# benanil/CLRayTracer

Hardware: AMD Instinct MI355X
Metric: Mrays/s (primary + traced secondary rays), ms/frame at 1920x1080 (higher is better)
Workload: dtype f32

## Files before the change

clraytracer_amd/_lib.py:

```python
import ctypes as C
import os

import numpy as np

os.environ.setdefault("GPU_MAX_HW_QUEUES", "8")

_HERE = os.path.dirname(os.path.abspath(__file__))
ROOT = os.path.dirname(_HERE)
HIP_SO = os.path.join(_HERE, "csrc", "libcrt_hip.so")
HOST_SO = os.path.join(_HERE, "host", "libcrt_host.so")


class CrtTraceArgs(C.Structure):
    _fields_ = [("cameraPos", C.c_float * 3), ("time", C.c_float), ("numMeshes", C.c_uint32), ("sunAngle", C.c_float)]


class CrtFrameStats(C.Structure):
    _fields_ = [("frames", C.c_uint64), ("sumMs", C.c_double * 4), ("extentMs", C.c_double), ("firstFrameMs", C.c_double)]


class CrtCounters(C.Structure):
    _fields_ = [(n, C.c_uint64) for n in ("rays", "primary", "secondary", "hits", "misses", "traversals", "pops",
                                          "innerVisits", "triTests", "capHits", "stackOverflows", "maxStack",
                                          "shadowRays", "shadowHits")]
# ... 22 lines not shown

HIP_API = {
    "crt_init": (C.c_int, [C.c_int, C.c_int, C.c_int]),
    "crt_init_devices": (C.c_int, [C.POINTER(C.c_int), C.c_int, C.c_int, C.c_int]),
    "crt_init_gpus": (C.c_int, [C.c_int, C.c_int, C.c_int]),
    "crt_num_devices": (C.c_int, []),
    "crt_peer_access": (C.c_int, [C.c_int]),
    "crt_gather_path": (C.c_char_p, []),
    "crt_get_cull_range": (C.c_int, [_fp, C.c_int, _fp, _fp, C.POINTER(C.c_uint64)]),
    "crt_debug_staggered_frames": (C.c_int, [C.POINTER(C.c_uint64)]),
    "crt_debug_inject_failure": (C.c_int, [C.c_int]),
    "crt_debug_last_kernel": (C.c_int, [C.c_char_p, C.c_size_t]),
    "crt_debug_last_gather": (C.c_int, [C.POINTER(C.c_uint64), C.POINTER(C.c_int)]),
    "crt_debug_build_stats": (C.c_int, [C.POINTER(C.c_uint32), C.POINTER(C.c_uint32)]),
    "crt_debug_tlas_stats": (C.c_int, [C.POINTER(C.c_uint64), C.POINTER(C.c_uint32), C.POINTER(C.c_uint32)]),
    "crt_debug_measure_clock": (C.c_int, [C.c_int, C.POINTER(C.c_double)]),
    "crt_shutdown": (C.c_int, []),
    "crt_resize": (C.c_int, [C.c_int, C.c_int]),
    "crt_set_row_bands": (C.c_int, [C.c_int, C.c_int, C.c_int]),
    "crt_row_owner": (C.c_int, [C.c_int, C.c_int, C.c_int]),
    "crt_band_plan": (C.c_int, [C.c_int, C.c_int, C.c_int, C.c_int, C.POINTER(C.c_int)]),
    "crt_upload_triangles": (C.c_int, [_vp, _sz, _sz]),
    "crt_upload_bvh_nodes": (C.c_int, [_vp, _sz, _sz]),
    "crt_upload_bvh_roots": (C.c_int, [_vp, _sz, _sz]),
    "crt_upload_materials": (C.c_int, [_vp, _sz, _sz]),
    "crt_upload_texture_table": (C.c_int, [_vp, _sz]),
    "crt_upload_texels": (C.c_int, [_vp, _sz, _sz]),
    "crt_upload_instances": (C.c_int, [_vp, _sz, _sz]),
    "crt_build_bvh": (C.c_int, [_sz, _vp, C.c_int, _sz, _sz, C.POINTER(C.c_uint32)]),
    "crt_download_triangles": (C.c_int, [_vp, _sz, _sz]),
# ... 148 lines not shown
```

clraytracer_amd/csrc/crt_device.h:

```cpp
#pragma once
#include <hip/hip_runtime.h>
#include <hip/hip_fp16.h>
#include <stdint.h>
#include "../../include/crt_types.h"

#define CRT_LEAF_BIT 0x80000000u
#define CRT_TOP_BIT 0x40000000u
#define CRT_BLOCK 64
#ifndef CRT_WAVES_PER_SIMD
#define CRT_WAVES_PER_SIMD 8
#endif
#define CRT_WAVES_PER_SIMD_COUNT 6
typedef uint32_t __attribute__((address_space(3))) * crt_lds_u32_ptr;
typedef float crt_f32x4 __attribute__((ext_vector_type(4)));
typedef const crt_f32x4 __attribute__((address_space(4)))* crt_const_f32x4_ptr;
typedef const crt_f32x4 __attribute__((address_space(3)))* crt_lds_f32x4_ptr;
#ifndef CRT_LDS_SLOTS
#define CRT_LDS_SLOTS 20
#endif
#define CRT_MAX_PARK 5
#define CRT_OVF_SLOTS_MAX (CRT_STACK_DEPTH - (CRT_LDS_SLOTS - CRT_MAX_PARK))
#define CRT_OVF_WORDS_PER_BLOCK ((size_t)CRT_OVF_SLOTS_MAX * CRT_BLOCK)
template <int PARK, int SLOTS = CRT_LDS_SLOTS, bool TOP = false>
struct CrtStackT {
    static constexpr bool kTop = TOP;
    static constexpr int kLds = SLOTS - PARK;
    static_assert(PARK >= 0 && PARK <= CRT_MAX_PARK && kLds >= 1 && kLds <= CRT_STACK_DEPTH && CRT_STACK_DEPTH - kLds <= CRT_OVF_SLOTS_MAX, "LDS slots");
    crt_lds_u32_ptr lds;
    uint32_t* ovf;
    crt_lds_f32x4_ptr top;
    uint32_t vblock;
    __device__ __forceinline__ uint32_t* overflow_slot(int k) const
    {
        uint32_t lane = threadIdx.x & 63;
        asm volatile("" : "+v"(lane));
        return ovf + ((size_t)(TOP ? vblock : blockIdx.x) * CRT_OVF_SLOTS_MAX + (size_t)k) * CRT_BLOCK + lane;
    }
    __device__ __forceinline__ void write(int slot, uint32_t v) const
    {
        const int s = slot & (CRT_STACK_DEPTH - 1);
        if (kLds >= CRT_STACK_DEPTH || __ballot(s >= kLds) == 0) { lds[s * 64] = v; return; }
        if (kLds >= CRT_STACK_DEPTH || s < kLds) lds[s * 64] = v;
        else *overflow_slot(s - kLds) = v;
    }
    __device__ __forceinline__ uint32_t read(int slot) const
    {
        const int s = slot & (CRT_STACK_DEPTH - 1);
        if (kLds >= CRT_STACK_DEPTH || __ballot(s >= kLds) == 0) return lds[s * 64];
        if (kLds >= CRT_STACK_DEPTH || s < kLds) return lds[s * 64];
        return *overflow_slot(s - kLds);
    }
    __device__ __forceinline__ crt_lds_f32x4_ptr top_record(uint32_t k) const { return top + k * 4; }
    __device__ __forceinline__ void park(int k, uint32_t v) const { lds[(kLds + k) * 64] = v; }
    __device__ __forceinline__ uint32_t parked(int k) const { return lds[(kLds + k) * 64]; }
};
typedef CrtStackT<0> CrtStack;
#ifndef CRT_SPLIT_BETA
#define CRT_SPLIT_BETA 1.2f
#endif
#ifndef CRT_SPLIT_BETA_ASYNC
#define CRT_SPLIT_BETA_ASYNC 2.0f
#endif
#define CRT_MAX_SPLIT 96
#ifndef CRT_MAX_SPLIT_PIPELINED
#define CRT_MAX_SPLIT_PIPELINED 8
#endif
#define CRT_TILE 8

struct CrtTlasNode { float4 sphere; uint32_t left, right, pad0, pad1; };
// ... 9 lines not shown
    const uint32_t* __restrict__ rootRefs;
    uint32_t* stackOverflow;
    const CrtMeshInstance* __restrict__ instances;
    const struct CrtDevInstance* __restrict__ devInstances;
    const float4* __restrict__ instBounds;
    const CrtMaterial* __restrict__ materials;
    const CrtTexture* __restrict__ textures;
    const uint32_t* __restrict__ texels;
    int numTexels;
    uint32_t numInstances;
    const CrtTlasNode* __restrict__ tlas;
    uint32_t tlasNodes;
    const uint32_t* __restrict__ alwaysList;
    uint32_t numAlways;
    const float4* __restrict__ topPairs;
};

struct CrtFrame {
    float invView[16];
    float invProj[16];
    float camPos[3];
    float lightY, lightZ;
    int width, height;
    int tilesX;
    int ownedTileRows;
    int gridBlocks;
    int tileRowsPerBand;
    int rank, nRanks;
    int slotsPerXcd;
    const uint32_t* order;
// ... 132 lines not shown
{
    CrtDevInstance I;
    const uint32_t inst0 = (uint32_t)__builtin_amdgcn_readfirstlane((int)inst);
    if (__ballot(inst != inst0) == 0) {
        const crt_const_f32x4_ptr p = (crt_const_f32x4_ptr)(table + inst0);
        const crt_f32x4 a = p[0], b = p[1], c = p[2], e = p[3];
        I.r0 = make_float4(a.x, a.y, a.z, a.w); I.r1 = make_float4(b.x, b.y, b.z, b.w);
        I.r2 = make_float4(c.x, c.y, c.z, c.w); I.r3 = make_float4(e.x, e.y, e.z, e.w);
    } else {
        const CrtDevInstance* ip = table + inst;
        I.r0 = ip->r0; I.r1 = ip->r1; I.r2 = ip->r2; I.r3 = ip->r3;
    }
    return I;
}

template <bool COUNT>
struct Traversal {
    v3 mo, md, inv;
    Triout tr;
    int sp, prot, inters;
    uint32_t ref, curInst;
    bool active;

    __device__ __forceinline__ void reset()
    {
        mo = mk3(0.f, 0.f, 0.f); md = mo; inv = mo;
        tr.t = 0.f; tr.u = 0.f; tr.v = 0.f; tr.tri = 0;
        sp = 0; prot = 0; inters = 0; ref = 0; curInst = 0; active = false;
    }
    __device__ __forceinline__ bool at_inner() const { return active && !(ref & CRT_LEAF_BIT); }
    __device__ __forceinline__ bool at_leaf() const { return active && (ref & CRT_LEAF_BIT); }

    __device__ __forceinline__ void finish(Closest& c)
    {
        if (inters) { c.hitInstance = (int)curInst; c.hit = tr; c.distance = tr.t; c.anyHit = 1; }
        active = false;
    }
    template <class STK>
    __device__ __forceinline__ void pop_next(const STK& stack, Closest& c, LaneCounters& lc)
    {
        const bool nonEmpty = sp > 0, canPop = nonEmpty && prot < CRT_MAX_POPS;
        prot += nonEmpty ? 1 : 0;
        if (COUNT) { if (nonEmpty && !canPop) lc.capHits++; if (canPop) lc.pops++; }
        if (canPop) { --sp; ref = stack.read(sp); }
        else {
            const bool keep = inters != 0;
            c.hitInstance = keep ? (int)curInst : c.hitInstance; c.distance = keep ? tr.t : c.distance; c.anyHit = keep ? 1 : c.anyHit;
            c.hit.t = keep ? tr.t : c.hit.t; c.hit.u = keep ? tr.u : c.hit.u; c.hit.v = keep ? tr.v : c.hit.v; c.hit.tri = keep ? tr.tri : c.hit.tri;
            active = false;
        }
    }
    template <bool TOP = false>
    __device__ __forceinline__ void enter(const CrtDevScene& S, uint32_t inst, v3 o, v3 d, float bestSoFar, LaneCounters& lc)
    {
        curInst = inst;
        const CrtDevInstance I = load_instance(S.devInstances, inst);
        mo = xform_xyz(I, o.x, o.y, o.z, 1.0f);
        md = xform_xyz(I, d.x, d.y, d.z, 0.0f);
        inv = mk3(1.0f / md.x, 1.0f / md.y, 1.0f / md.z);
        tr.t = bestSoFar; tr.tri = 0; tr.u = 0.0f; tr.v = 0.0f;
        ref = __float_as_uint(TOP ? I.r2.w : I.r0.w);
        sp = 0; prot = 1; inters = 0; active = true;
        if (COUNT) { lc.traversals++; lc.pops++; }
    }
    template <class STK>
    __device__ __forceinline__ void inner(const CrtDevScene& S, const STK& stack, Closest& c, LaneCounters& lc)
    {
        float dist1, dist2;
        uint32_t nearRef, farRef;
        const uint32_t ref0 = (uint32_t)__builtin_amdgcn_readfirstlane((int)ref);
        if (__ballot(ref != ref0) == 0) {
            const crt_const_f32x4_ptr q = (STK::kTop && (ref0 & CRT_TOP_BIT)) ? (crt_const_f32x4_ptr)(S.topPairs + (size_t)(ref0 & 0xFFFFu) * 4)
                                                                             : (crt_const_f32x4_ptr)(S.pairs + (size_t)ref0 * 4);
            const crt_f32x4 a = q[0], b = q[1], c4 = q[2], e = q[3];
            dist1 = intersect_aabb(mo, inv, make_float4(a.x, a.y, a.z, a.w), make_float4(b.x, b.y, b.z, b.w), tr.t);
            dist2 = intersect_aabb(mo, inv, make_float4(c4.x, c4.y, c4.z, c4.w), make_float4(e.x, e.y, e.z, e.w), tr.t);
            nearRef = __float_as_uint(a.w); farRef = __float_as_uint(c4.w);
#ifndef CRT_TOP_NO_LDS_PATH
#define CRT_TOP_NO_LDS_PATH 0
#endif
// ... 6 lines not shown
        } else {
            const float4* p = (STK::kTop && (ref & CRT_TOP_BIT)) ? S.topPairs + (size_t)(ref & 0xFFFFu) * 4 : S.pairs + (size_t)ref * 4;
            const float4 lmin = p[0], lmax = p[1], rmin = p[2], rmax = p[3];
            dist1 = intersect_aabb(mo, inv, lmin, lmax, tr.t);
            dist2 = intersect_aabb(mo, inv, rmin, rmax, tr.t);
            nearRef = __float_as_uint(lmin.w); farRef = __float_as_uint(rmin.w);
        }
        if (COUNT) lc.innerVisits++;
        {
            const bool sw = dist1 > dist2;
            const float d1 = sw ? dist2 : dist1, d2 = sw ? dist1 : dist2;
            const uint32_t r1 = sw ? farRef : nearRef, r2 = sw ? nearRef : farRef;
            dist1 = d1; dist2 = d2; nearRef = r1; farRef = r2;
        }
        if (dist2 != 1e30f) {
            if (COUNT) { if (sp >= CRT_STACK_DEPTH) lc.stackOverflows++; }
            stack.write(sp, farRef);
            sp++;
            if (COUNT) { if ((uint32_t)sp > lc.maxStack) lc.maxStack = (uint32_t)sp; }
        }
        if (dist1 == 1e30f) pop_next(stack, c, lc);
        else ref = nearRef;
    }
    template <bool ANYHIT, class STK>
    __device__ __forceinline__ void leaf(const CrtDevScene& S, const STK& stack, Closest& c, LaneCounters& lc)
    {
        const uint32_t first = ref & 0x00FFFFFFu;
        uint32_t n = (ref >> 24) & 0x7Fu;
        if (n == 0) n = S.bigLeaf[first];
        for (uint32_t i = first, end = first + n; i < end; ++i) {
            if (COUNT) lc.triTests++;
            const float* __restrict__ hot = S.triHot + (size_t)i * 9;
            inters |= intersect_triangle(mo, md, mk3(hot[0], hot[1], hot[2]), mk3(hot[3], hot[4], hot[5]), mk3(hot[6], hot[7], hot[8]), tr, i);
            if (ANYHIT) { if (inters) break; }
        }
        if (ANYHIT && inters) finish(c);
        else pop_next(stack, c, lc);
    }
};

__device__ __forceinline__ bool sphere_culls(const float4 bs, v3 o, v3 d, float dd)
{
    const v3 oc = mk3(bs.x - o.x, bs.y - o.y, bs.z - o.z);
    const float oc2 = dot3(oc, oc), b = dot3(oc, d);
    const float r2 = bs.w * bs.w * 1.0201f + 4e-6f * oc2;
    return (bs.w >= 0.0f) & ((oc2 * dd - b * b > r2 * dd) | ((b < 0.0f) & (oc2 > r2)));
}

template <bool COUNT, bool DEFER_COUNT = false>
__device__ __forceinline__ unsigned long long candidate_mask(const CrtDevScene& S, v3 o, v3 d, uint32_t base, uint32_t cnt, LaneCounters& lc)
{
    const float dd = dot3(d, d);
// ... 48 lines not shown
    uint32_t node = 0; int sp = 0;
    for (;;) {
        const CrtTlasNode nd = S.tlas[node];
        bool descend = false;
        if (!sphere_culls(nd.sphere, o, d, dd)) {
            if (nd.left & CRT_TLAS_LEAF) {
                const uint32_t i = nd.left & 0xFFFFu;
                if (i < S.numInstances) ok = candidate_list_add(stack, n, i) && ok;
            } else { stack.write(sp, nd.right); sp++; node = nd.left; descend = true; }
        }
        if (!descend) { if (sp == 0) break; --sp; node = stack.read(sp); }
    }
    return ok;
}

template <bool COUNT, bool ITERS, bool ANYHIT, class STK>
__device__ __forceinline__ void trip_steps(const CrtDevScene& S, const STK& stack, Traversal<COUNT>& T, Closest& c, LaneCounters& lc, bool done)
{
    if (!done && T.at_inner()) {
        if (ITERS) { lc.rays++; if (first_active_lane()) lc.innerVisits++; }
        T.inner(S, stack, c, lc);
    }
    if (!done && T.at_leaf()) {
        if (ITERS) {
            if (first_active_lane()) lc.triTests++;
            uint32_t n = (T.ref >> 24) & 0x7Fu; if (n == 0) n = S.bigLeaf[T.ref & 0x00FFFFFFu];
            for (int off = 32; off > 0; off >>= 1) { const uint32_t o2 = (uint32_t)__shfl_xor((int)n, off, 64); n = o2 > n ? o2 : n; }
            if (first_active_lane()) lc.misses += n;
        }
        T.template leaf<ANYHIT>(S, stack, c, lc);
    }
    if (!done && T.at_inner()) {
        if (ITERS) { if (first_active_lane()) lc.hits++; }
        T.inner(S, stack, c, lc);
    }
}

template <bool COUNT, bool ITERS = false, bool ANYHIT = false, bool TLAS = false, class STK = CrtStack>
__device__ __forceinline__ Closest closest_hit(const CrtDevScene& S, v3 o, v3 d, const STK& stack, LaneCounters& lc)
{
    Closest c = no_hit();
    Traversal<COUNT> T; T.reset();

    if constexpr (TLAS) {
        static_assert(!TLAS || STK::kLds <= CRT_LDS_SLOTS - CRT_TLAS_PARK, "the candidate list needs CRT_TLAS_PARK parked slots");
        uint32_t listed = 0;
        const bool fits = tlas_candidates(S, o, d, stack, listed);
        if (__ballot(!fits) == 0) {
            int prev = -1;
            if (COUNT && !ANYHIT) { const uint32_t culled = S.numInstances - listed; lc.traversals += culled; lc.pops += culled; lc.innerVisits += culled; lc.culled += culled; }
            bool done = false;
            for (;;) {
                const bool wEnter = !done && !T.active;
                const bool wInner = !done && T.at_inner();
                const bool wLeaf = !done && T.at_leaf();
                if (__ballot(wEnter || wInner || wLeaf) == 0) break;
                if (wEnter) {
                    const uint32_t k = (ANYHIT && c.anyHit) ? 0xFFFFu : candidate_list_next(stack, prev);
                    if (k == 0xFFFFu) {
                        done = true;
                        if (COUNT && ANYHIT && !c.anyHit) { const uint32_t n = S.numInstances - (uint32_t)(prev + 1); lc.traversals += n; lc.pops += n; lc.innerVisits += n; lc.culled += n; }
                    } else {
                        if (COUNT && ANYHIT) { const uint32_t n = k - (uint32_t)(prev + 1); lc.traversals += n; lc.pops += n; lc.innerVisits += n; lc.culled += n; }
                        prev = (int)k;
                        T.template enter<STK::kTop>(S, k, o, d, c.distance, lc);
                    }
                }
                trip_steps<COUNT, false, ANYHIT>(S, stack, T, c, lc, done);
            }
            return c;
        }
    }

    for (uint32_t base = 0; base < S.numInstances; base += 64) {
        const uint32_t cnt = (S.numInstances - base) < 64u ? (S.numInstances - base) : 64u;
        unsigned long long cand = candidate_mask<COUNT, ANYHIT>(S, o, d, base, cnt, lc);
        unsigned long long culledLeft = (COUNT && ANYHIT) ? (~cand & (cnt == 64u ? ~0ull : ((1ull << cnt) - 1ull))) : 0ull;
        bool done = ANYHIT && c.anyHit;
        for (;;) {
            const bool wEnter = !done && !T.active;
            const bool wInner = !done && T.at_inner();
            const bool wLeaf = !done && T.at_leaf();
            if (__ballot(wEnter || wInner || wLeaf) == 0) break;
// ... 3 lines not shown
                else if (cand == 0) {
                    done = true;
                    if (COUNT && ANYHIT) { const uint32_t n = (uint32_t)__popcll(culledLeft); lc.traversals += n; lc.pops += n; lc.innerVisits += n; lc.culled += n; culledLeft = 0; }
                } else {
                    if (ITERS) { if (first_active_lane()) lc.traversals++; }
                    const uint32_t k = (uint32_t)__ffsll((long long)cand) - 1u;
                    cand &= cand - 1;
                    if (COUNT && ANYHIT) {
                        const unsigned long long below = culledLeft & ((1ull << k) - 1ull);
                        const uint32_t n = (uint32_t)__popcll(below);
                        lc.traversals += n; lc.pops += n; lc.innerVisits += n; lc.culled += n; culledLeft &= ~below;
                    }
                    T.template enter<STK::kTop>(S, base + k, o, d, c.distance, lc);
                }
            }
            trip_steps<COUNT, ITERS, ANYHIT>(S, stack, T, c, lc, done);
        }
    }
    return c;
}

__device__ __forceinline__ int clamp_texel(int idx, int n) { return idx < 0 ? 0 : (idx >= n ? n - 1 : idx); }

__device__ __noinline__ int sample_skybox(v3 d, int texW, int texH)
{
    const double PI = 3.14159265358979323846;
    float at = (float)(atan2((double)d.x, (double)(-d.z)) / PI);
    float ac = (float)(acos((double)d.y) / PI);
    int theta = f2i((at * 0.5f) * (float)texW);
    int phi = f2i(ac * (float)texH);
    return (int)((uint32_t)phi * (uint32_t)texW + (uint32_t)(theta + 2));
// ... 128 lines not shown
```

clraytracer_amd/csrc/crt_instances.h:

```cpp
#pragma once
namespace {

int cache_root_nodes();
void rebuild_instance_master(uint32_t dirtyFirst = 0, uint32_t dirtyCount = CRT_MAX_INSTANCES, bool everything = true);

int rebuild_bvh_layout()
{
    HIPCHK(hipMemsetAsync(g.err, 0, sizeof(int), g.stream));
    if (g.nodeCount) {
        crt_relayout_nodes<<<(g.nodeCount + 255) / 256, 256, 0, g.stream>>>(g.rawNodes, g.nodeCount, (uint32_t)g.triCap, g.pairs, g.bigLeaf, g.err);
        HIPCHK(hipGetLastError());
    }
    crt_make_root_refs<<<(CRT_MAX_MESHES + 255) / 256, 256, 0, g.stream>>>(g.rawNodes, g.nodeCount, (uint32_t)g.triCap, g.roots, g.numRoots, g.rootRefs, g.bigLeaf, g.err);
    HIPCHK(hipGetLastError());
    {
        const uint32_t perMesh = g.numRoots ? (uint32_t)CRT_TOP_PAIRS / g.numRoots : 0u;
        crt_build_top_kernel<<<1, CRT_MAX_MESHES, 0, g.stream>>>(g.pairs, g.rootRefs, g.numRoots, perMesh, g.topPairs, g.topRootRefs);
        HIPCHK(hipGetLastError());
    }
    int err = 0;
    HIPCHK(hipMemcpyAsync(&err, g.err, sizeof(int), hipMemcpyDeviceToHost, g.stream));
    HIPCHK(hipStreamSynchronize(g.stream));
    g.sceneValid = (err == 0);
    if (err) return CRT_E_BAD_ARGUMENT;
    RCCHK(cache_root_nodes());
    rebuild_instance_master();
    return CRT_OK;
}

bool invert4(const double m[16], double out[16])
{
    double a[4][8];
    for (int r = 0; r < 4; ++r) for (int c = 0; c < 4; ++c) { a[r][c] = m[r * 4 + c]; a[r][4 + c] = (r == c) ? 1.0 : 0.0; }
    for (int col = 0; col < 4; ++col) {
        int piv = col;
        for (int r = col + 1; r < 4; ++r) if (fabs(a[r][col]) > fabs(a[piv][col])) piv = r;
        if (!(fabs(a[piv][col]) > 1e-300)) return false;
// ... 212 lines not shown
```

clraytracer_amd/csrc/crt_kernels.h:

```cpp
#pragma once
#include "crt_device.h"

__device__ __forceinline__ uint32_t wave_sum(uint32_t v)
{
    for (int off = 32; off > 0; off >>= 1) v += __shfl_xor(v, off, 64);
    return v;
}
__device__ __forceinline__ uint32_t wave_max(uint32_t v)
{
    for (int off = 32; off > 0; off >>= 1) { uint32_t o = __shfl_xor(v, off, 64); v = o > v ? o : v; }
    return v;
}

__device__ __forceinline__ void flush_counters(const LaneCounters& lc, unsigned long long* g)
{
    uint32_t s[14] = { lc.rays, lc.primary, lc.secondary, lc.hits, lc.misses, lc.traversals, lc.pops,
                       lc.innerVisits, lc.triTests, lc.capHits, lc.stackOverflows, lc.shadowRays, lc.shadowHits, lc.culled };
    uint32_t mx = wave_max(lc.maxStack);
#pragma unroll
    for (int k = 0; k < 14; ++k) {
        uint32_t t = wave_sum(s[k]);
        if ((threadIdx.x & 63) == 0 && t) atomicAdd(&g[k < 11 ? k : k + 1], (unsigned long long)t);
    }
    if ((threadIdx.x & 63) == 0) atomicMax(&g[11], (unsigned long long)mx);
// ... 275 lines not shown
            if ((lane & (k * k - 1)) == 0) {
                const int sh = k == 4 ? 2 : 1;
                int w2 = F.width >> sh, h2 = F.height >> sh;
                asm volatile("" : "+s"(w2), "+s"(h2));
                finish_pixel(F, rgb, qx >> sh, qy >> sh, w2, h2, out);
            }
        } else {
            lane_pixel_again(F, b, lane, qx, qy);
            int w2 = F.width, h2 = F.height;
            asm volatile("" : "+s"(w2), "+s"(h2));
            finish_pixel(F, ps.result, qx, qy, w2, h2, out);
        }
    }
    add_tile_cost(F, costSlot, tc0, isQuadrant);
    if (COUNT) flush_counters(lc, counters);
    if (STAMP) write_wave_stamp(counters, lc, t0);
}

template <bool COUNT, bool STAMP = false, bool SHADOW = false, bool TLAS = false, bool REFRACT = false>
__global__ __launch_bounds__(CRT_BLOCK, (COUNT || STAMP) ? CRT_WAVES_PER_SIMD_COUNT : CRT_WAVES_PER_SIMD)
void crt_trace_kernel(CrtDevScene S, CrtFrame F, float4* __restrict__ out, unsigned long long* __restrict__ counters)
{
    __shared__ uint32_t s_stack[CRT_LDS_SLOTS * CRT_BLOCK];
    const CrtTraceStack<SHADOW, TLAS> stack = { (crt_lds_u32_ptr)s_stack + threadIdx.x, S.stackOverflow };
    trace_body<COUNT, STAMP, SHADOW, TLAS, REFRACT, false>(S, F, out, counters, stack, blockIdx.x, (int)(threadIdx.x & 63));
}

template <bool COUNT, bool SHADOW, bool TLAS, bool REFRACT>
__global__ __launch_bounds__(CRT_BLOCK, COUNT ? CRT_WAVES_PER_SIMD_COUNT - 1 : CRT_WAVES_PER_SIMD)
void crt_trace_ssaa_kernel(CrtDevScene S, CrtFrame F, float4* __restrict__ out, unsigned long long* __restrict__ counters)
{
// ... 224 lines not shown
```

clraytracer_amd/csrc/crt_refill.h:

```cpp
#pragma once
#include "crt_kernels.h"

#ifndef CRT_REFILL_TILES
#define CRT_REFILL_TILES 2
#endif
#ifndef CRT_REFILL_BATCH
#define CRT_REFILL_BATCH 32
#endif
#ifndef CRT_REFILL_RATIO
#define CRT_REFILL_RATIO 1
#endif
#define CRT_REFILL_PIXELS (64 * CRT_REFILL_TILES)

__device__ __forceinline__ bool refill_block(const CrtFrame& F, int b, int& tx0, int& tileRow, int& costSlot, int tiles = CRT_REFILL_TILES)
{
    int bx = 0, quadrant;
    const bool dealt = deal_tile(F, b, bx, tileRow, quadrant, &costSlot);
    tx0 = bx * tiles;
    return dealt;
}

__device__ __forceinline__ void refill_pixel(int tx0, int tileRow, uint32_t p, int& px, int& py) { tile_pixel(tx0 + (int)(p >> 6), tileRow, (int)(p & 63u), px, py); }

template <bool COUNT, bool STAMP = false>
// ... 1 lines not shown
void crt_trace_refill_kernel(CrtDevScene S, CrtFrame F, float4* __restrict__ out, unsigned long long* __restrict__ counters)
{
    __shared__ uint32_t s_stack[CRT_LDS_SLOTS * CRT_BLOCK];
    typedef CrtStackT<2> Stack;
    const Stack stack = { (crt_lds_u32_ptr)s_stack + threadIdx.x, S.stackOverflow };
    LaneCounters lc; zero_counters(lc);
    WaveStampStart t0 = { 0, 0 };
    if (STAMP) t0 = wave_stamp_start();
    const unsigned long long tc0 = tile_cost_start(F);
    int tx0 = 0, tileRow = 0, costSlot = -1;
    const bool valid = refill_block(F, blockIdx.x, tx0, tileRow, costSlot);
    if (valid) {
        uint32_t cursor = 0;
        PathState ps = camera_path(F, mk3(0.f, 0.f, 0.f));
        Closest c = no_hit();
        Traversal<COUNT> T; T.reset();
        unsigned long long cand = 0;
        bool havePath = false;
        const uint32_t cnt = S.numInstances < 64u ? S.numInstances : 64u;
        for (;;) {
            const bool rayDone = havePath && !T.active && cand == 0;
            const unsigned long long mDone = __ballot(rayDone);
            const unsigned long long mBusy = __ballot(havePath && !rayDone);
            if ((mDone | mBusy) == 0 && cursor >= (uint32_t)CRT_REFILL_PIXELS) break;
            const uint32_t nDone = (uint32_t)__popcll(mDone), nBusy = (uint32_t)__popcll(mBusy);
            if (STAMP) { if (first_active_lane()) lc.pops++; }
            if (nDone >= (uint32_t)CRT_REFILL_BATCH || (uint32_t)CRT_REFILL_RATIO * nDone > nBusy || nBusy == 0) {
                bool newRay = false;
                if (STAMP) { if (first_active_lane()) lc.capHits++; }
                if (rayDone) {
                    T.reset();
// ... 52 lines not shown
    if (STAMP) write_wave_stamp(counters, lc, t0, wave_sum(lc.capHits));
}

#ifndef CRT_BLOCK_TILES
#define CRT_BLOCK_TILES 2
#endif
#define CRT_BLOCK_PIXELS (64 * CRT_BLOCK_TILES)

template <bool COUNT, bool STAMP = false>
__global__ __launch_bounds__(CRT_BLOCK, (COUNT || STAMP) ? CRT_WAVES_PER_SIMD_COUNT : CRT_WAVES_PER_SIMD)
void crt_trace_block_kernel(CrtDevScene S, CrtFrame F, float4* __restrict__ out, unsigned long long* __restrict__ counters, CrtBounceRay* __restrict__ queue)
{
    __shared__ uint32_t s_stack[CRT_LDS_SLOTS * CRT_BLOCK];
    typedef CrtStackT<CRT_BLOCK_TILES> Stack;
    const Stack stack = { (crt_lds_u32_ptr)s_stack + threadIdx.x, S.stackOverflow };
    const crt_lds_u32_ptr list = (crt_lds_u32_ptr)s_stack + Stack::kLds * 64;
    const uint32_t lane = threadIdx.x & 63u;
    LaneCounters lc; zero_counters(lc);
    WaveStampStart t0 = { 0, 0 };
    if (STAMP) t0 = wave_stamp_start();
    const unsigned long long tc0 = tile_cost_start(F);
    int tx0 = 0, tileRow = 0, costSlot = -1;
    const bool valid = refill_block(F, blockIdx.x, tx0, tileRow, costSlot, CRT_BLOCK_TILES);
    if (valid) {
        const uint32_t cnt = S.numInstances < 64u ? S.numInstances : 64u;
        CrtBounceRay* __restrict__ q = queue + (size_t)costSlot * CRT_BLOCK_PIXELS;
        uint32_t nList = 0, nQueue = 0;
        for (uint32_t t = 0; t < (uint32_t)CRT_BLOCK_TILES; ++t) {
            const uint32_t p = t * 64u + lane;
            int px, py;
            refill_pixel(tx0, tileRow, p, px, py);
// ... 71 lines not shown
```

clraytracer_amd/csrc/crt_relayout.h:

```cpp
#pragma once
#include "crt_device.h"

__global__ void crt_relayout_tris(const CrtTri* __restrict__ raw, size_t first, size_t count,
                                  float* __restrict__ hot, uint4* __restrict__ cold)
{
    size_t k = (size_t)blockIdx.x * blockDim.x + threadIdx.x;
    if (k >= count) return;
    const size_t i = first + k;
    const CrtTri t = raw[i];
    float* h = hot + i * 9;
    h[0] = t.v0[0]; h[1] = t.v0[1]; h[2] = t.v0[2];
    h[3] = t.v1[0] - t.v0[0]; h[4] = t.v1[1] - t.v0[1]; h[5] = t.v1[2] - t.v0[2];
    h[6] = t.v2[0] - t.v0[0]; h[7] = t.v2[1] - t.v0[1]; h[8] = t.v2[2] - t.v0[2];
    const uint4* tail = reinterpret_cast<const uint4*>(reinterpret_cast<const char*>(raw + i) + 48);
    cold[i * 2] = tail[0];
    cold[i * 2 + 1] = tail[1];
}

__global__ void crt_tri_reach_kernel(const CrtTri* __restrict__ raw, size_t first, size_t count, uint32_t* __restrict__ reachBits)
{
    const size_t k = (size_t)blockIdx.x * blockDim.x + threadIdx.x;
    float m = 0.0f;
    if (k < count) {
        const CrtTri t = raw[first + k];
// ... 30 lines not shown
    if (n >= nodeCount) return;
    const CrtBVHNode node = raw[n];
    if (node.triCount > 0) return;
    const uint32_t l = node.leftFirst;
    if (l <= n || (uint64_t)l + 1 >= (uint64_t)nodeCount) { atomicOr(err, 2); return; }
    const CrtBVHNode L = raw[l], R = raw[l + 1];
    const uint32_t lref = make_ref(L, l, nodeCount, triCap, bigLeaf, err);
    const uint32_t rref = make_ref(R, l + 1, nodeCount, triCap, bigLeaf, err);
    float4* p = pairs + (size_t)(l >> 1) * 4;
    p[0] = make_float4(L.aabbMin[0], L.aabbMin[1], L.aabbMin[2], __uint_as_float(lref));
    p[1] = make_float4(L.aabbMax[0], L.aabbMax[1], L.aabbMax[2], 0.0f);
    p[2] = make_float4(R.aabbMin[0], R.aabbMin[1], R.aabbMin[2], __uint_as_float(rref));
    p[3] = make_float4(R.aabbMax[0], R.aabbMax[1], R.aabbMax[2], 0.0f);
}

__global__ void crt_make_root_refs(const CrtBVHNode* __restrict__ raw, uint32_t nodeCount, uint32_t triCap,
                                   const uint32_t* __restrict__ roots, uint32_t numRoots,
                                   uint32_t* __restrict__ rootRefs, uint32_t* __restrict__ bigLeaf, int* __restrict__ err)
{
    uint32_t k = blockIdx.x * blockDim.x + threadIdx.x;
    if (k >= CRT_MAX_MESHES) return;
    const uint32_t r = k < numRoots ? roots[k] : 0xFFFFFFFFu;
    if (r >= nodeCount) { rootRefs[k] = crt_empty_ref(triCap); return; }
    rootRefs[k] = make_ref(raw[r], r, nodeCount, triCap, bigLeaf, err);
}

__global__ void crt_refresh_instances_kernel(const uint4* __restrict__ staging, uint4* __restrict__ block, uint32_t words16,
                                             const uint32_t* __restrict__ rootRefs, const uint32_t* __restrict__ topRootRefs,
                                             uint32_t count, CrtDevInstance* __restrict__ out)
{
// ... 22 lines not shown
```

clraytracer_amd/csrc/crt_shim.hip:

```cpp
#include <hip/hip_runtime.h>
#include <math.h>
#include <stdio.h>
#include <string.h>
#include <stdlib.h>
#include "../../include/crt_api.h"
#include "../../include/crt_debug.h"
#include "crt_kernels.h"
#include "crt_refill.h"
#include "crt_ldstop.h"
#include "crt_relayout.h"
#include "crt_bvh_build.h"
#include <vector>
#include <algorithm>
#include <utility>
#include <thread>
#include <mutex>
#include <condition_variable>
#include <functional>
#include <atomic>
#include "crt_state.h"
#include "crt_instances.h"
#include "crt_upload.h"
#include "crt_bvh_driver.h"
#include "crt_frame.h"
// ... 101 lines not shown
    { const char* e = getenv("CRT_DEBUG_HOOKS"); if (!e || atoi(e) == 0) return CRT_E_UNSUPPORTED; }
    if (device < 0 || device >= M.n) return CRT_E_BAD_ARGUMENT;
    M.injectFailure = device;
    return CRT_OK;
}
int crt_debug_staggered_frames(uint64_t* out) { NEED_SESSION(); if (!out) return CRT_E_BAD_ARGUMENT; Use u_(0); *out = g.staggeredFrames; return CRT_OK; }
int crt_debug_tlas_stats(uint64_t* builds, uint32_t* refitsSinceBuild, uint32_t* nodes)
{
    NEED_SESSION();
    Use u_(0);
    if (builds) *builds = g.hTlasBuilds;
    if (refitsSinceBuild) *refitsSinceBuild = g.hTlasRefits;
    if (nodes) *nodes = g.hTlasNodes;
    return CRT_OK;
}
int crt_debug_build_stats(uint32_t* levels, uint32_t* launches)
{
    NEED_SESSION();
    Use u_(0);
    if (levels) *levels = g.buildLevels;
    if (launches) *launches = g.buildLaunches;
    return CRT_OK;
}
int crt_debug_last_gather(uint64_t* bytes, int* bytesPerPixel)
{
    NEED_SESSION();
    if (bytes) *bytes = M.n > 1 ? M.lastGatherBytes : 0;
    if (bytesPerPixel) *bytesPerPixel = M.n > 1 ? M.lastGatherBpp : 0;
    return CRT_OK;
}
// ... 150 lines not shown
```

clraytracer_amd/csrc/crt_state.h:

```cpp
#pragma once
namespace {

#define CRT_MAX_FRAMES_IN_FLIGHT 8
#define CRT_MAX_DEVICES 16

enum class Form { Mega, Wavefront, Refill, Block, LdsTop };

struct EventSet {
    hipEvent_t ev[4] = { nullptr, nullptr, nullptr, nullptr };
    bool pending = false; int flags = 0; bool evRaygen = false, evPost = false;
    unsigned long long seq = 0;
};

struct FrameSlot {
    hipStream_t stream = nullptr;
    EventSet es[2];
    unsigned frames = 0;
    float4* out = nullptr;
    float4* aux = nullptr; size_t auxPixels = 0;
    CrtBounceRay* blockQueue = nullptr; size_t blockQueueCap = 0;
    uint32_t* wfCount = nullptr; size_t wfCap = 0;
    uint32_t* ovf = nullptr; size_t ovfWords = 0;
    uint32_t* lists = nullptr; size_t listsCap = 0;
    int orderSlots = -1; int orderKey[7] = { 0, 0, 0, 0, 0, 0, 0 };
// ... 50 lines not shown
    float lastView[35] = { 0 }; unsigned long long lastViewInst = 0; bool viewMoved = false;
    float splitBeta = CRT_SPLIT_BETA, splitBetaAsync = CRT_SPLIT_BETA_ASYNC;
    Form form = Form::Mega;
    float4* topPairs = nullptr; uint32_t* topRootRefs = nullptr;
    char lastKernel[128] = { 0 };
    char* queryBuf = nullptr; size_t queryBytes = 0;
    void* buildBuf = nullptr; size_t buildBytes = 0;
    std::vector<CrtBuildCtl> buildReplay; unsigned long long buildReplayKey = 0;
    unsigned buildLaunches = 0, buildLevels = 0;
    bool buildNoSpin = false;
    CrtBuildCtlHost* buildCtlHost = nullptr; uint32_t buildSeq = 0;
    CrtTri* buildTris = nullptr;
    size_t triCap = 0, nodeCap = 0, texelByteCap = 0;
    uint32_t nodeCount = 0, numRoots = 0; size_t texelBytesHigh = 0; size_t trisHigh = 0;
    bool sceneValid = true;
    double msSum[4] = { 0, 0, 0, 0 }; unsigned long long framesTimed = 0;
    float ms[4] = { 0, 0, 0, 0 }; unsigned long long msSeq = 0, frameSeq = 0;
    hipEvent_t statStart = nullptr; bool statStartArmed = true, statStartValid = false; unsigned long long statStartSeq = 0; double statExtent = 0, statFirstMs = 0;
    CrtCounters lastCounters; unsigned long long lastCulled = 0;
    double frameLog[512]; unsigned frameLogN = 0;
    State* primary = nullptr; State* group[CRT_MAX_DEVICES] = { nullptr }; int groupSize = 1;
    int gather8 = 1;
};
thread_local State* G = nullptr;
#define g (*G)

static inline void crt_cpu_relax()
{
#if defined(__x86_64__) || defined(__i386__)
    __builtin_ia32_pause();
// ... 65 lines not shown
    }
    F.width = ss * g.width; F.height = ss * g.height; F.ss = ss;
    set_tile_grid(F, owned_tile_rows(F.height, ss * g.bandRows), (F.width + CRT_TILE - 1) / CRT_TILE);
    F.tileRowsPerBand = ss * g.bandRows / CRT_TILE;
    F.rank = g.rank; F.nRanks = g.nRanks;
}

void fill_scene(CrtDevScene& S, uint32_t numInstances, const FrameSlot& fs, bool noCull = false)
{
    S.pairs = g.pairs; S.triHot = g.triHot; S.triCold = g.triCold; S.bigLeaf = g.bigLeaf; S.rootRefs = g.rootRefs; S.stackOverflow = fs.ovf;
    S.instances = fs.instances; S.devInstances = fs.devInstances; S.instBounds = fs.instBounds; S.materials = g.materials; S.textures = g.textures; S.texels = g.texels;
    S.numTexels = (int)((g.texelBytesHigh + 2) / 3);
    if (S.numTexels < 1) S.numTexels = 1;
    S.numInstances = numInstances;
    S.tlas = fs.tlas; S.tlasNodes = fs.tlasNodes; S.alwaysList = fs.alwaysList; S.numAlways = fs.numAlways;
    S.topPairs = g.topPairs;
    if (noCull) { S.instBounds = g.noCullBounds; S.tlas = nullptr; S.tlasNodes = 0; S.alwaysList = nullptr; S.numAlways = 0; g.noCullFrames++; }
}
bool beyond_cull_range(double originNorm) { return !(originNorm <= (double)g.cullOriginLimit); }

int ensure_overflow(FrameSlot& fs, size_t blocks) { return grow(fs.ovf, fs.ovfWords, blocks * CRT_OVF_WORDS_PER_BLOCK, fs.stream); }

int alloc_frame_buffers(int w, int h)
{
    const size_t pixels = (size_t)w * (size_t)h;
    float* rays = nullptr; float4* outs[CRT_MAX_FRAMES_IN_FLIGHT] = {};
    hipError_t e = hipMalloc(&rays, sizeof(float) * 3 * pixels);
    for (int i = 0; i < g.nSlots && e == hipSuccess; ++i) {
        e = hipMalloc(&outs[i], sizeof(float4) * pixels);
        if (e == hipSuccess) e = hipMemsetAsync(outs[i], 0, sizeof(float4) * pixels, g.stream);
    }
// ... 48 lines not shown
```

include/crt_debug.h:

```cpp
#ifndef CRT_DEBUG_H
#define CRT_DEBUG_H
#include "crt_api.h"
#ifdef __cplusplus
extern "C" {
#endif

int crt_debug_read_stamps(uint64_t* dst, size_t maxWaves, size_t* numWaves);
int crt_debug_read_frame_times(double* dst, size_t maxFrames, size_t* numFrames);
int crt_debug_measure_clock(int micros, double* ghz);
int crt_debug_inject_failure(int device);
int crt_debug_staggered_frames(uint64_t* out);

int crt_debug_last_kernel(char* dst, size_t cap);
int crt_debug_last_gather(uint64_t* bytes, int* bytesPerPixel);
int crt_debug_build_stats(uint32_t* levels, uint32_t* launches);
int crt_debug_tlas_stats(uint64_t* builds, uint32_t* refitsSinceBuild, uint32_t* nodes);

#ifdef __cplusplus
}
#endif
#endif
```

Before: 10550.

## Store truncated push distances in LDS and skip popped nodes beyond closest hit

```diff
diff --git a/clraytracer_amd/_lib.py b/clraytracer_amd/_lib.py
--- a/clraytracer_amd/_lib.py
+++ b/clraytracer_amd/_lib.py
@@ -60,6 +60,7 @@
     "crt_debug_last_gather": (C.c_int, [C.POINTER(C.c_uint64), C.POINTER(C.c_int)]),
     "crt_debug_build_stats": (C.c_int, [C.POINTER(C.c_uint32), C.POINTER(C.c_uint32)]),
     "crt_debug_tlas_stats": (C.c_int, [C.POINTER(C.c_uint64), C.POINTER(C.c_uint32), C.POINTER(C.c_uint32)]),
+    "crt_debug_pop_skip": (C.c_int, [C.POINTER(C.c_uint32)]),
     "crt_debug_measure_clock": (C.c_int, [C.c_int, C.POINTER(C.c_double)]),
     "crt_shutdown": (C.c_int, []),
     "crt_resize": (C.c_int, [C.c_int, C.c_int]),
diff --git a/clraytracer_amd/csrc/crt_device.h b/clraytracer_amd/csrc/crt_device.h
--- a/clraytracer_amd/csrc/crt_device.h
+++ b/clraytracer_amd/csrc/crt_device.h
@@ -12,6 +12,7 @@
 #endif
 #define CRT_WAVES_PER_SIMD_COUNT 6
 typedef uint32_t __attribute__((address_space(3))) * crt_lds_u32_ptr;
+typedef uint16_t __attribute__((address_space(3))) * crt_lds_u16_ptr;
 typedef float crt_f32x4 __attribute__((ext_vector_type(4)));
 typedef const crt_f32x4 __attribute__((address_space(4)))* crt_const_f32x4_ptr;
 typedef const crt_f32x4 __attribute__((address_space(3)))* crt_lds_f32x4_ptr;
@@ -19,13 +20,15 @@
 #define CRT_LDS_SLOTS 20
 #endif
 #define CRT_MAX_PARK 5
-#define CRT_OVF_SLOTS_MAX (CRT_STACK_DEPTH - (CRT_LDS_SLOTS - CRT_MAX_PARK))
+#define CRT_LDS_ENTRIES(rows) ((rows) * 4 / 6)
+#define CRT_OVF_SLOTS_MAX (CRT_STACK_DEPTH - CRT_LDS_ENTRIES(CRT_LDS_SLOTS - CRT_MAX_PARK))
 #define CRT_OVF_WORDS_PER_BLOCK ((size_t)CRT_OVF_SLOTS_MAX * CRT_BLOCK)
 template <int PARK, int SLOTS = CRT_LDS_SLOTS, bool TOP = false>
 struct CrtStackT {
     static constexpr bool kTop = TOP;
-    static constexpr int kLds = SLOTS - PARK;
-    static_assert(PARK >= 0 && PARK <= CRT_MAX_PARK && kLds >= 1 && kLds <= CRT_STACK_DEPTH && CRT_STACK_DEPTH - kLds <= CRT_OVF_SLOTS_MAX, "LDS slots");
+    static constexpr int kRows = SLOTS - PARK;
+    static constexpr int kLds = CRT_LDS_ENTRIES(kRows);
+    static_assert(PARK >= 0 && PARK <= CRT_MAX_PARK && kLds >= 1 && kLds + (kLds + 1) / 2 <= kRows && kLds <= CRT_STACK_DEPTH && CRT_STACK_DEPTH - kLds <= CRT_OVF_SLOTS_MAX, "LDS slots");
     crt_lds_u32_ptr lds;
     uint32_t* ovf;
     crt_lds_f32x4_ptr top;
@@ -36,6 +39,11 @@
         asm volatile("" : "+v"(lane));
         return ovf + ((size_t)(TOP ? vblock : blockIdx.x) * CRT_OVF_SLOTS_MAX + (size_t)k) * CRT_BLOCK + lane;
     }
+    __device__ __forceinline__ crt_lds_u16_ptr code_slot(int s) const
+    {
+        asm volatile("" : "+v"(s));
+        return (crt_lds_u16_ptr)(lds + (kLds + (s >> 1)) * 64) + (s & 1);
+    }
     __device__ __forceinline__ void write(int slot, uint32_t v) const
     {
         const int s = slot & (CRT_STACK_DEPTH - 1);
@@ -50,9 +58,24 @@
         if (kLds >= CRT_STACK_DEPTH || s < kLds) return lds[s * 64];
         return *overflow_slot(s - kLds);
     }
+    __device__ __forceinline__ void push(int slot, uint32_t v, uint32_t code) const
+    {
+        const int s = slot & (CRT_STACK_DEPTH - 1);
+        if (kLds >= CRT_STACK_DEPTH || __ballot(s >= kLds) == 0) { lds[s * 64] = v; *code_slot(s) = (uint16_t)code; return; }
+        if (kLds >= CRT_STACK_DEPTH || s < kLds) { lds[s * 64] = v; *code_slot(s) = (uint16_t)code; }
+        else *overflow_slot(s - kLds) = v;
+    }
+    __device__ __forceinline__ uint32_t pop(int slot, uint32_t& code) const
+    {
+        const int s = slot & (CRT_STACK_DEPTH - 1);
+        if (kLds >= CRT_STACK_DEPTH || __ballot(s >= kLds) == 0) { code = *code_slot(s); return lds[s * 64]; }
+        if (kLds >= CRT_STACK_DEPTH || s < kLds) { code = *code_slot(s); return lds[s * 64]; }
+        code = 0;
+        return *overflow_slot(s - kLds);
+    }
     __device__ __forceinline__ crt_lds_f32x4_ptr top_record(uint32_t k) const { return top + k * 4; }
-    __device__ __forceinline__ void park(int k, uint32_t v) const { lds[(kLds + k) * 64] = v; }
-    __device__ __forceinline__ uint32_t parked(int k) const { return lds[(kLds + k) * 64]; }
+    __device__ __forceinline__ void park(int k, uint32_t v) const { lds[(kRows + k) * 64] = v; }
+    __device__ __forceinline__ uint32_t parked(int k) const { return lds[(kRows + k) * 64]; }
 };
 typedef CrtStackT<0> CrtStack;
 #ifndef CRT_SPLIT_BETA
@@ -92,6 +115,7 @@
     const uint32_t* __restrict__ alwaysList;
     uint32_t numAlways;
     const float4* __restrict__ topPairs;
+    uint32_t popSkip;
 };
 
 struct CrtFrame {
@@ -254,11 +278,11 @@
     return I;
 }
 
-template <bool COUNT>
+template <bool COUNT, bool ITERS = false>
 struct Traversal {
     v3 mo, md, inv;
     Triout tr;
-    int sp, prot, inters;
+    uint32_t sps;
     uint32_t ref, curInst;
     bool active;
 
@@ -266,25 +290,46 @@
     {
         mo = mk3(0.f, 0.f, 0.f); md = mo; inv = mo;
         tr.t = 0.f; tr.u = 0.f; tr.v = 0.f; tr.tri = 0;
-        sp = 0; prot = 0; inters = 0; ref = 0; curInst = 0; active = false;
-    }
+        sps = 0; ref = 0; curInst = 0; active = false;
+    }
+    __device__ __forceinline__ int sp() const { return (int)(sps & 0xFFFFu); }
+    __device__ __forceinline__ bool inters() const { return (sps >> 31) != 0; }
     __device__ __forceinline__ bool at_inner() const { return active && !(ref & CRT_LEAF_BIT); }
     __device__ __forceinline__ bool at_leaf() const { return active && (ref & CRT_LEAF_BIT); }
 
     __device__ __forceinline__ void finish(Closest& c)
     {
-        if (inters) { c.hitInstance = (int)curInst; c.hit = tr; c.distance = tr.t; c.anyHit = 1; }
+        if (inters()) { c.hitInstance = (int)curInst; c.hit = tr; c.distance = tr.t; c.anyHit = 1; }
         active = false;
     }
-    template <class STK>
+    template <bool SKIP = true, class STK>
     __device__ __forceinline__ void pop_next(const STK& stack, Closest& c, LaneCounters& lc)
     {
-        const bool nonEmpty = sp > 0, canPop = nonEmpty && prot < CRT_MAX_POPS;
-        prot += nonEmpty ? 1 : 0;
-        if (COUNT) { if (nonEmpty && !canPop) lc.capHits++; if (canPop) lc.pops++; }
-        if (canPop) { --sp; ref = stack.read(sp); }
-        else {
-            const bool keep = inters != 0;
+        bool canPop, again;
+        uint32_t skipped = 0;
+        do {
+            const bool nonEmpty = sp() > 0;
+            canPop = nonEmpty && (sps & 0x7FFFFFFFu) < ((uint32_t)CRT_MAX_POPS << 16);
+            sps += nonEmpty ? 0x10000u : 0u;
+            again = false;
+            if (canPop) {
+                --sps;
+                if (SKIP) {
+                    uint32_t code;
+                    ref = stack.pop((int)sps, code);
+                    again = !(ref & CRT_LEAF_BIT) && code != 0 && !(__uint_as_float(code << 16) < tr.t);
+                } else ref = stack.read((int)sps);
+            }
+            skipped += again ? 1 : 0;
+        } while (SKIP && again);
+        if (COUNT) {
+            if (sp() > 0 && !canPop) lc.capHits++;
+            lc.pops += skipped + (canPop ? 1 : 0);
+            lc.innerVisits += skipped;
+        }
+        if (ITERS) lc.culled += skipped;
+        if (!canPop) {
+            const bool keep = inters();
             c.hitInstance = keep ? (int)curInst : c.hitInstance; c.distance = keep ? tr.t : c.distance; c.anyHit = keep ? 1 : c.anyHit;
             c.hit.t = keep ? tr.t : c.hit.t; c.hit.u = keep ? tr.u : c.hit.u; c.hit.v = keep ? tr.v : c.hit.v; c.hit.tri = keep ? tr.tri : c.hit.tri;
             active = false;
@@ -300,10 +345,10 @@
         inv = mk3(1.0f / md.x, 1.0f / md.y, 1.0f / md.z);
         tr.t = bestSoFar; tr.tri = 0; tr.u = 0.0f; tr.v = 0.0f;
         ref = __float_as_uint(TOP ? I.r2.w : I.r0.w);
-        sp = 0; prot = 1; inters = 0; active = true;
+        sps = 1u << 16; active = true;
         if (COUNT) { lc.traversals++; lc.pops++; }
     }
-    template <class STK>
+    template <bool SKIP = true, class STK>
     __device__ __forceinline__ void inner(const CrtDevScene& S, const STK& stack, Closest& c, LaneCounters& lc)
     {
         float dist1, dist2;
@@ -340,15 +385,16 @@
             dist1 = d1; dist2 = d2; nearRef = r1; farRef = r2;
         }
         if (dist2 != 1e30f) {
-            if (COUNT) { if (sp >= CRT_STACK_DEPTH) lc.stackOverflows++; }
-            stack.write(sp, farRef);
-            sp++;
-            if (COUNT) { if ((uint32_t)sp > lc.maxStack) lc.maxStack = (uint32_t)sp; }
-        }
-        if (dist1 == 1e30f) pop_next(stack, c, lc);
+            if (COUNT) { if (sp() >= CRT_STACK_DEPTH) lc.stackOverflows++; }
+            if (SKIP) stack.push((int)sps, farRef, __float_as_uint(dist2) >> (S.popSkip ? 16u : 31u));
+            else stack.write((int)sps, farRef);
+            sps++;
+            if (COUNT) { if ((uint32_t)sp() > lc.maxStack) lc.maxStack = (uint32_t)sp(); }
+        }
+        if (dist1 == 1e30f) pop_next<SKIP>(stack, c, lc);
         else ref = nearRef;
     }
-    template <bool ANYHIT, class STK>
+    template <bool ANYHIT, bool SKIP = !ANYHIT, class STK>
     __device__ __forceinline__ void leaf(const CrtDevScene& S, const STK& stack, Closest& c, LaneCounters& lc)
     {
         const uint32_t first = ref & 0x00FFFFFFu;
@@ -357,11 +403,11 @@
         for (uint32_t i = first, end = first + n; i < end; ++i) {
             if (COUNT) lc.triTests++;
             const float* __restrict__ hot = S.triHot + (size_t)i * 9;
-            inters |= intersect_triangle(mo, md, mk3(hot[0], hot[1], hot[2]), mk3(hot[3], hot[4], hot[5]), mk3(hot[6], hot[7], hot[8]), tr, i);
-            if (ANYHIT) { if (inters) break; }
-        }
-        if (ANYHIT && inters) finish(c);
-        else pop_next(stack, c, lc);
+            sps |= (uint32_t)intersect_triangle(mo, md, mk3(hot[0], hot[1], hot[2]), mk3(hot[3], hot[4], hot[5]), mk3(hot[6], hot[7], hot[8]), tr, i) << 31;
+            if (ANYHIT) { if (inters()) break; }
+        }
+        if (ANYHIT && inters()) finish(c);
+        else pop_next<SKIP>(stack, c, lc);
     }
 };
 
@@ -440,12 +486,12 @@
     return ok;
 }
 
-template <bool COUNT, bool ITERS, bool ANYHIT, class STK>
-__device__ __forceinline__ void trip_steps(const CrtDevScene& S, const STK& stack, Traversal<COUNT>& T, Closest& c, LaneCounters& lc, bool done)
+template <bool COUNT, bool ITERS, bool ANYHIT, bool SKIP = !ANYHIT, class STK>
+__device__ __forceinline__ void trip_steps(const CrtDevScene& S, const STK& stack, Traversal<COUNT, ITERS>& T, Closest& c, LaneCounters& lc, bool done)
 {
     if (!done && T.at_inner()) {
         if (ITERS) { lc.rays++; if (first_active_lane()) lc.innerVisits++; }
-        T.inner(S, stack, c, lc);
+        T.template inner<SKIP>(S, stack, c, lc);
     }
     if (!done && T.at_leaf()) {
         if (ITERS) {
@@ -454,22 +500,24 @@
             for (int off = 32; off > 0; off >>= 1) { const uint32_t o2 = (uint32_t)__shfl_xor((int)n, off, 64); n = o2 > n ? o2 : n; }
             if (first_active_lane()) lc.misses += n;
         }
-        T.template leaf<ANYHIT>(S, stack, c, lc);
+        T.template leaf<ANYHIT, SKIP>(S, stack, c, lc);
     }
     if (!done && T.at_inner()) {
         if (ITERS) { if (first_active_lane()) lc.hits++; }
-        T.inner(S, stack, c, lc);
+        T.template inner<SKIP>(S, stack, c, lc);
     }
 }
 
 template <bool COUNT, bool ITERS = false, bool ANYHIT = false, bool TLAS = false, class STK = CrtStack>
 __device__ __forceinline__ Closest closest_hit(const CrtDevScene& S, v3 o, v3 d, const STK& stack, LaneCounters& lc)
 {
+    static_assert(!(TLAS && ITERS), "the stamped launch has no instance-tree form");
+    constexpr bool kSkip = !ANYHIT && !TLAS;
     Closest c = no_hit();
-    Traversal<COUNT> T; T.reset();
+    Traversal<COUNT, ITERS> T; T.reset();
 
     if constexpr (TLAS) {
-        static_assert(!TLAS || STK::kLds <= CRT_LDS_SLOTS - CRT_TLAS_PARK, "the candidate list needs CRT_TLAS_PARK parked slots");
+        static_assert(!TLAS || STK::kRows <= CRT_LDS_SLOTS - CRT_TLAS_PARK, "the candidate list needs CRT_TLAS_PARK parked slots");
         uint32_t listed = 0;
         const bool fits = tlas_candidates(S, o, d, stack, listed);
         if (__ballot(!fits) == 0) {
@@ -492,7 +540,7 @@
                         T.template enter<STK::kTop>(S, k, o, d, c.distance, lc);
                     }
                 }
-                trip_steps<COUNT, false, ANYHIT>(S, stack, T, c, lc, done);
+                trip_steps<COUNT, ITERS, ANYHIT, kSkip>(S, stack, T, c, lc, done);
             }
             return c;
         }
@@ -526,7 +574,7 @@
                     T.template enter<STK::kTop>(S, base + k, o, d, c.distance, lc);
                 }
             }
-            trip_steps<COUNT, ITERS, ANYHIT>(S, stack, T, c, lc, done);
+            trip_steps<COUNT, ITERS, ANYHIT, kSkip>(S, stack, T, c, lc, done);
         }
     }
     return c;
diff --git a/clraytracer_amd/csrc/crt_instances.h b/clraytracer_amd/csrc/crt_instances.h
--- a/clraytracer_amd/csrc/crt_instances.h
+++ b/clraytracer_amd/csrc/crt_instances.h
@@ -9,6 +9,8 @@
     HIPCHK(hipMemsetAsync(g.err, 0, sizeof(int), g.stream));
     if (g.nodeCount) {
         crt_relayout_nodes<<<(g.nodeCount + 255) / 256, 256, 0, g.stream>>>(g.rawNodes, g.nodeCount, (uint32_t)g.triCap, g.pairs, g.bigLeaf, g.err);
+        HIPCHK(hipGetLastError());
+        crt_check_nesting_kernel<<<(g.nodeCount + 255) / 256, 256, 0, g.stream>>>(g.rawNodes, g.nodeCount, g.pairs, g.err);
         HIPCHK(hipGetLastError());
     }
     crt_make_root_refs<<<(CRT_MAX_MESHES + 255) / 256, 256, 0, g.stream>>>(g.rawNodes, g.nodeCount, (uint32_t)g.triCap, g.roots, g.numRoots, g.rootRefs, g.bigLeaf, g.err);
@@ -21,6 +23,8 @@
     int err = 0;
     HIPCHK(hipMemcpyAsync(&err, g.err, sizeof(int), hipMemcpyDeviceToHost, g.stream));
     HIPCHK(hipStreamSynchronize(g.stream));
+    g.popSkip = (err & CRT_ERR_NOT_NESTED) ? 0u : 1u;
+    err &= ~CRT_ERR_NOT_NESTED;
     g.sceneValid = (err == 0);
     if (err) return CRT_E_BAD_ARGUMENT;
     RCCHK(cache_root_nodes());
diff --git a/clraytracer_amd/csrc/crt_kernels.h b/clraytracer_amd/csrc/crt_kernels.h
--- a/clraytracer_amd/csrc/crt_kernels.h
+++ b/clraytracer_amd/csrc/crt_kernels.h
@@ -313,7 +313,7 @@
     }
     add_tile_cost(F, costSlot, tc0, isQuadrant);
     if (COUNT) flush_counters(lc, counters);
-    if (STAMP) write_wave_stamp(counters, lc, t0);
+    if (STAMP) write_wave_stamp(counters, lc, t0, wave_sum(lc.culled));
 }
 
 template <bool COUNT, bool STAMP = false, bool SHADOW = false, bool TLAS = false, bool REFRACT = false>
diff --git a/clraytracer_amd/csrc/crt_refill.h b/clraytracer_amd/csrc/crt_refill.h
--- a/clraytracer_amd/csrc/crt_refill.h
+++ b/clraytracer_amd/csrc/crt_refill.h
@@ -39,7 +39,7 @@
         uint32_t cursor = 0;
         PathState ps = camera_path(F, mk3(0.f, 0.f, 0.f));
         Closest c = no_hit();
-        Traversal<COUNT> T; T.reset();
+        Traversal<COUNT, STAMP> T; T.reset();
         unsigned long long cand = 0;
         bool havePath = false;
         const uint32_t cnt = S.numInstances < 64u ? S.numInstances : 64u;
@@ -122,7 +122,7 @@
     __shared__ uint32_t s_stack[CRT_LDS_SLOTS * CRT_BLOCK];
     typedef CrtStackT<CRT_BLOCK_TILES> Stack;
     const Stack stack = { (crt_lds_u32_ptr)s_stack + threadIdx.x, S.stackOverflow };
-    const crt_lds_u32_ptr list = (crt_lds_u32_ptr)s_stack + Stack::kLds * 64;
+    const crt_lds_u32_ptr list = (crt_lds_u32_ptr)s_stack + Stack::kRows * 64;
     const uint32_t lane = threadIdx.x & 63u;
     LaneCounters lc; zero_counters(lc);
     WaveStampStart t0 = { 0, 0 };
diff --git a/clraytracer_amd/csrc/crt_relayout.h b/clraytracer_amd/csrc/crt_relayout.h
--- a/clraytracer_amd/csrc/crt_relayout.h
+++ b/clraytracer_amd/csrc/crt_relayout.h
@@ -68,6 +68,36 @@
     p[3] = make_float4(R.aabbMax[0], R.aabbMax[1], R.aabbMax[2], 0.0f);
 }
 
+__device__ __forceinline__ bool crt_box_nests(const float4 cmin, const float4 cmax, const float4 pmin, const float4 pmax)
+{
+    const float big = 3.402823466e38f;
+    return pmin.x <= cmin.x && cmin.x <= cmax.x && cmax.x <= pmax.x && pmin.y <= cmin.y && cmin.y <= cmax.y && cmax.y <= pmax.y &&
+           pmin.z <= cmin.z && cmin.z <= cmax.z && cmax.z <= pmax.z &&
+           fabsf(pmin.x) <= big && fabsf(pmin.y) <= big && fabsf(pmin.z) <= big && fabsf(pmax.x) <= big && fabsf(pmax.y) <= big && fabsf(pmax.z) <= big;
+}
+
+#define CRT_ERR_NOT_NESTED 4
+__global__ void crt_check_nesting_kernel(const CrtBVHNode* __restrict__ raw, uint32_t nodeCount, const float4* __restrict__ pairs, int* __restrict__ err)
+{
+    const uint32_t n = blockIdx.x * blockDim.x + threadIdx.x;
+    if (n >= nodeCount) return;
+    const CrtBVHNode node = raw[n];
+    if (node.triCount > 0) return;
+    const uint32_t l = node.leftFirst;
+    if (l <= n || (uint64_t)l + 1 >= (uint64_t)nodeCount) return;
+    const float4* p = pairs + (size_t)(l >> 1) * 4;
+    bool nested = true;
+    for (int side = 0; side < 2; ++side) {
+        const float4 bmin = p[side * 2], bmax = p[side * 2 + 1];
+        const uint32_t ref = __float_as_uint(bmin.w);
+        if (ref & CRT_LEAF_BIT) continue;
+        if ((uint64_t)ref * 2 + 1 >= (uint64_t)nodeCount) { nested = false; continue; }
+        const float4* q = pairs + (size_t)ref * 4;
+        nested = nested && crt_box_nests(q[0], q[1], bmin, bmax) && crt_box_nests(q[2], q[3], bmin, bmax);
+    }
+    if (!nested) atomicOr(err, CRT_ERR_NOT_NESTED);
+}
+
 __global__ void crt_make_root_refs(const CrtBVHNode* __restrict__ raw, uint32_t nodeCount, uint32_t triCap,
                                    const uint32_t* __restrict__ roots, uint32_t numRoots,
                                    uint32_t* __restrict__ rootRefs, uint32_t* __restrict__ bigLeaf, int* __restrict__ err)
diff --git a/clraytracer_amd/csrc/crt_shim.hip b/clraytracer_amd/csrc/crt_shim.hip
--- a/clraytracer_amd/csrc/crt_shim.hip
+++ b/clraytracer_amd/csrc/crt_shim.hip
@@ -139,6 +139,7 @@
     if (nodes) *nodes = g.hTlasNodes;
     return CRT_OK;
 }
+int crt_debug_pop_skip(uint32_t* on) { NEED_SESSION(); if (!on) return CRT_E_BAD_ARGUMENT; Use u_(0); *on = g.popSkip; return CRT_OK; }
 int crt_debug_build_stats(uint32_t* levels, uint32_t* launches)
 {
     NEED_SESSION();
diff --git a/clraytracer_amd/csrc/crt_state.h b/clraytracer_amd/csrc/crt_state.h
--- a/clraytracer_amd/csrc/crt_state.h
+++ b/clraytracer_amd/csrc/crt_state.h
@@ -88,6 +88,7 @@
     size_t triCap = 0, nodeCap = 0, texelByteCap = 0;
     uint32_t nodeCount = 0, numRoots = 0; size_t texelBytesHigh = 0; size_t trisHigh = 0;
     bool sceneValid = true;
+    uint32_t popSkip = 0;
     double msSum[4] = { 0, 0, 0, 0 }; unsigned long long framesTimed = 0;
     float ms[4] = { 0, 0, 0, 0 }; unsigned long long msSeq = 0, frameSeq = 0;
     hipEvent_t statStart = nullptr; bool statStartArmed = true, statStartValid = false; unsigned long long statStartSeq = 0; double statExtent = 0, statFirstMs = 0;
@@ -183,7 +184,7 @@
     if (S.numTexels < 1) S.numTexels = 1;
     S.numInstances = numInstances;
     S.tlas = fs.tlas; S.tlasNodes = fs.tlasNodes; S.alwaysList = fs.alwaysList; S.numAlways = fs.numAlways;
-    S.topPairs = g.topPairs;
+    S.topPairs = g.topPairs; S.popSkip = g.popSkip;
     if (noCull) { S.instBounds = g.noCullBounds; S.tlas = nullptr; S.tlasNodes = 0; S.alwaysList = nullptr; S.numAlways = 0; g.noCullFrames++; }
 }
 bool beyond_cull_range(double originNorm) { return !(originNorm <= (double)g.cullOriginLimit); }
diff --git a/include/crt_debug.h b/include/crt_debug.h
--- a/include/crt_debug.h
+++ b/include/crt_debug.h
@@ -15,6 +15,7 @@
 int crt_debug_last_gather(uint64_t* bytes, int* bytesPerPixel);
 int crt_debug_build_stats(uint32_t* levels, uint32_t* launches);
 int crt_debug_tlas_stats(uint64_t* builds, uint32_t* refitsSinceBuild, uint32_t* nodes);
+int crt_debug_pop_skip(uint32_t* on);
 
 #ifdef __cplusplus
 }
```

Measured after the change: 8878. -15.8%, worse.
